# Borx25/CPU-Raytracing-experiments

Hardware: AMD Instinct MI355X
Metric: Mray/s (primary+bounce) (higher is better)
Workload: dtype f32; 1 GPU; cfg4: 4096x4096 px, S(100000) spheres + SAH BVH, MIS, Policy.max_bounces=9 (primary+8 bounces), 5 buckets, 64 accumulations/step; fixed image, tile rows split over the GPUs; image=4096x4096, spheres=100000, max_bounces=9, buckets=5, parallelism=single GPU, batches_in_flight=1, accumulations_per_batch=63, accumulations_per_batch_limit=63

## Files before the change

### cpu-raytracing-experiments_amd/csrc/kernels.hpp

```cpp
#pragma once
#include <hip/hip_runtime.h>
#include <stdint.h>
#include "device_math.hpp"

namespace mirt {

constexpr uint32_t kBlock = 256;
constexpr uint32_t kShadeBlock = 512;
constexpr uint32_t kTraceBlock = 1024;
constexpr uint32_t kLdsStack = 16;
constexpr uint32_t kLdsStackWide = 12;
constexpr uint32_t kLeafBit = 0x80000000u;
constexpr uint32_t kTileSize = 256;
constexpr uint32_t kTileRoot = 16;
constexpr uint32_t kStack = 64;
constexpr uint32_t kDestAccum = 0x80000000u;

struct SceneDev {
	const float4* recs;
	const float4* spheres;
	const int32_t* prim_mat;
	const float4* light_sphere;
	const float4* light_emit;
	const float4* mat_albedo;
// ... 6 lines not shown
	uint32_t wide;
	uint32_t chunk_max;
	uint32_t leaf_batch;
	uint32_t refill_idle;
	uint32_t stack16;
	float ambient[3];
	int32_t hdri_w, hdri_h;
	float hdri_fw, hdri_fh;
	uint32_t has_ambient;
	uint32_t use_bvh;
};

struct StreamBuf {
	float *px, *py, *pz, *dx, *dy, *dz;
	float *tr, *tg, *tb;
	float *rr, *rg, *rb;
	uint32_t* path;
};
struct ShadowBuf {
	float *px, *py, *pz;
	float *dx, *dy, *dz, *tfar;
	float *sr, *sg, *sb;
	float *rr, *rg, *rb;
	float *er, *eg, *eb;
	uint32_t* dest;
};
struct FrameParams {
	CameraParams cam;
	uint32_t h_tiles;
	uint32_t first_tile;
	uint32_t run_tiles;
	uint32_t stride_tiles;
	uint32_t n_pix;
	uint32_t pix_bits;
	uint32_t pix_mask;
	uint32_t acc_base;
	uint32_t batch_n;
	uint32_t idx_base;
	uint32_t idx_buckets;
	uint32_t max_bounces;
	uint32_t buckets;
	uint32_t mis;
	uint32_t n_lights;
	uint32_t first_groups;
	float inv_n_pix, inv_h_tiles, inv_run_tiles;
};
struct alignas(8) HitRec { float tfar; int32_t prim; };
struct DevCounters {
	unsigned long long rays, shadow_rays, nodes, spheres, shadow_nodes, shadow_spheres, terminated, dropped;
};

MIRT_DI uint32_t lane_id() { return __builtin_amdgcn_mbcnt_hi(~0u, __builtin_amdgcn_mbcnt_lo(~0u, 0u)); }
MIRT_DI uint32_t mask_rank(unsigned long long m) {
	return __builtin_amdgcn_mbcnt_hi(static_cast<uint32_t>(m >> 32), __builtin_amdgcn_mbcnt_lo(static_cast<uint32_t>(m), 0u));
// ... 526 lines not shown
	const bool all = bvh_all_in_lds(sc);
	if (sc.half_boxes && sc.wide) {
		if (!sc.stack16) trace_persistent<MODE, COUNT, false, true, false, true>(sc, tl, q, n, work_next, fat, c_nodes, c_spheres, load_ray, store_result, col);
		else if (all) trace_persistent<MODE, COUNT, true, true, true, true>(sc, tl, q, n, work_next, fat, c_nodes, c_spheres, load_ray, store_result, col);
		else trace_persistent<MODE, COUNT, false, true, true, true>(sc, tl, q, n, work_next, fat, c_nodes, c_spheres, load_ray, store_result, col);
	} else if (sc.half_boxes) {
		if (!sc.stack16) trace_persistent<MODE, COUNT, false, true, false, false>(sc, tl, q, n, work_next, fat, c_nodes, c_spheres, load_ray, store_result, col);
		else if (all) trace_persistent<MODE, COUNT, true, true, true, false>(sc, tl, q, n, work_next, fat, c_nodes, c_spheres, load_ray, store_result, col);
		else trace_persistent<MODE, COUNT, false, true, true, false>(sc, tl, q, n, work_next, fat, c_nodes, c_spheres, load_ray, store_result, col);
	} else {
		if (all) trace_persistent<MODE, COUNT, true, false, false, false>(sc, tl, q, n, work_next, fat, c_nodes, c_spheres, load_ray, store_result, col);
		else trace_persistent<MODE, COUNT, false, false, false, false>(sc, tl, q, n, work_next, fat, c_nodes, c_spheres, load_ray, store_result, col);
	}
}

MIRT_DI size_t accum_index(uint32_t acc_base, uint32_t buckets, uint32_t pix_bits, uint32_t path) {
	const uint32_t slot = path >> pix_bits;
	const uint32_t pix = path & ((1u << pix_bits) - 1u);
	const uint32_t bucket = (acc_base + slot + 1u) % buckets;
	return (static_cast<size_t>(pix >> 8) * buckets + bucket) * 3u * kTileSize + (pix & 255u);
}
MIRT_DI size_t accum_index(const FrameParams& fp, uint32_t path) { return accum_index(fp.idx_base, fp.idx_buckets, fp.pix_bits, path); }
MIRT_DI void accumulate_add(float* __restrict__ accum, size_t idx, float r, float g, float b) {
	accum[idx] += r; accum[idx + kTileSize] += g; accum[idx + 2 * kTileSize] += b;
}
constexpr uint32_t kIdxContrib = 0xffffffffu;
MIRT_DI size_t contrib_index(uint32_t batch_n, uint32_t pix_bits, uint32_t path) {
	const uint32_t slot = path >> pix_bits;
	const uint32_t pix = path & ((1u << pix_bits) - 1u);
	return ((static_cast<size_t>(pix >> 8) * batch_n + slot) * kTileSize + (pix & 255u)) * 3u;
}
MIRT_DI void path_result(float* __restrict__ accum, uint32_t idx_base, uint32_t idx_buckets, uint32_t pix_bits, uint32_t path, float r, float g, float b) {
	if (idx_base == kIdxContrib) {
		float* w = accum + contrib_index(idx_buckets, pix_bits, path);
		w[0] = 0.0f + r; w[1] = 0.0f + g; w[2] = 0.0f + b;
	} else accumulate_add(accum, accum_index(idx_base, idx_buckets, pix_bits, path), r, g, b);
}
MIRT_DI void path_result_add(float* __restrict__ accum, uint32_t idx_base, uint32_t idx_buckets, uint32_t pix_bits, uint32_t path, float r, float g, float b) {
	if (idx_base == kIdxContrib) {
		float* w = accum + contrib_index(idx_buckets, pix_bits, path);
		w[0] += r; w[1] += g; w[2] += b;
	} else accumulate_add(accum, accum_index(idx_base, idx_buckets, pix_bits, path), r, g, b);
}
MIRT_DI void path_result(float* __restrict__ accum, const FrameParams& fp, uint32_t path, float r, float g, float b) { path_result(accum, fp.idx_base, fp.idx_buckets, fp.pix_bits, path, r, g, b); }
constexpr uint32_t kDestFull = 0x40000000u;
constexpr uint32_t kDestSlot = 0x3fffffffu;
struct ShadowSink {
	float *rr, *rg, *rb;
	const float *px, *py, *pz;
	float* accum;
	uint32_t acc_base, buckets, pix_bits;
	uint32_t* occ;
};
MIRT_DI void shadow_origin(const ShadowBuf& sh, const ShadowSink& sink, uint32_t i, float& px, float& py, float& pz) {
	if (sink.occ) { px = sh.px[i]; py = sh.py[i]; pz = sh.pz[i]; return; }
	const uint32_t dw = sh.dest[i];
	if (dw & kDestAccum) { px = sh.px[i]; py = sh.py[i]; pz = sh.pz[i]; }
	else { const uint32_t d = dw & kDestSlot; px = sink.px[d]; py = sink.py[d]; pz = sink.pz[d]; }
}
MIRT_DI void shadow_finish(const ShadowBuf& sh, const ShadowSink& sink, uint32_t i, bool occluded, uint32_t& c_term) {
	if (sink.occ) { sink.occ[i] = occluded ? 1u : 0u; return; }
	const uint32_t dw = sh.dest[i];
	const uint32_t dest = dw & (kDestSlot | kDestAccum);
	if (dw & kDestAccum) c_term++;
	if (dw & kDestFull) {
		f3 R{ sh.rr[i], sh.rg[i], sh.rb[i] };
		const f3 E{ sh.er[i], sh.eg[i], sh.eb[i] };
		if (!occluded) { R.x += sh.sr[i]; R.y += sh.sg[i]; R.z += sh.sb[i]; }
		R.x += E.x; R.y += E.y; R.z += E.z;
		if (dest & kDestAccum) path_result(sink.accum, sink.acc_base, sink.buckets, sink.pix_bits, dest & ~kDestAccum, R.x, R.y, R.z);
		else { sink.rr[dest] = R.x; sink.rg[dest] = R.y; sink.rb[dest] = R.z; }
	} else if (!occluded) {
		const f3 S{ sh.sr[i], sh.sg[i], sh.sb[i] };
		if (dest & kDestAccum) path_result_add(sink.accum, sink.acc_base, sink.buckets, sink.pix_bits, dest & ~kDestAccum, S.x, S.y, S.z);
		else { sink.rr[dest] += S.x; sink.rg[dest] += S.y; sink.rb[dest] += S.z; }
	}
}

constexpr int kPrimaryNone = 0, kPrimaryAll = 1, kPrimaryList = 2;
MIRT_DI uint32_t primary_list_ray(const FrameParams& fp, const uint32_t* __restrict__ ov_pix, uint32_t n_ov, float inv_n_ov, uint32_t j) {
	uint32_t k;
	const uint32_t slot = udiv_f(j, n_ov, inv_n_ov, k);
	return slot * fp.n_pix + ov_pix[k];
}
template <bool COUNT, int PRIMARY>
__global__ __launch_bounds__(kTraceBlock, 8) void k_trace(SceneDev sc, FrameParams fp,
                                                       StreamBuf in, HitRec* __restrict__ hit_out,
                                                       Queue closest_queue, uint32_t* closest_work,
                                                       ShadowBuf sh, ShadowSink sink,
                                                       Queue shadow_queue, uint32_t* shadow_work, FatList fat_closest, FatList fat_shadow,
                                                       DevCounters* ctr) {
// ... 186 lines not shown

MIRT_DI uint32_t block_compact(bool flag, uint32_t value, uint32_t* scratch, uint32_t* list) {
	const unsigned long long m = __ballot(flag);
	const uint32_t wave = threadIdx.x >> 6, n_waves = blockDim.x >> 6;
	if (lane_id() == 0) scratch[wave] = static_cast<uint32_t>(__popcll(m));
	__syncthreads();
	uint32_t before = 0, total = 0;
	for (uint32_t w = 0; w < n_waves; w++) { const uint32_t c = scratch[w]; before += (w < wave) ? c : 0u; total += c; }
	if (flag) list[before + mask_rank(m)] = value;
	__syncthreads();
	return total;
}

template <bool FIRST, bool GGX>
__global__ __launch_bounds__(kShadeBlock, 6) void k_shade(SceneDev sc, FrameParams fp, StreamBuf in, const HitRec* __restrict__ hit_in, StreamBuf out, ShadowBuf sh, uint32_t bounce,
                                                  Queue in_queue, Queue next_queue, Queue shadow_queue, float* __restrict__ accum, DevCounters* ctr,
                                                  const float4* __restrict__ mat_ggx, float gloss_decay) {
	const QueueView qin = FIRST ? queue_identity(fp.n_pix * fp.batch_n) : queue_view(in_queue);
	const uint32_t n = qin.pre[kSegs];
	const uint32_t n_chunks = (fp.n_pix + kShadeBlock - 1u) / kShadeBlock;
	const bool last_bounce = !(bounce < fp.max_bounces - 1u);
	const float light_selection_pdf = 1.0f / static_cast<float>(fp.n_lights);
	__shared__ uint32_t append_scratch[72];
	__shared__ uint32_t compact_scratch[17];
	__shared__ uint32_t hit_list[kShadeBlock];
	__shared__ float4 s_albedo[MIRT_MAX_MATERIALS + 1], s_emission[MIRT_MAX_MATERIALS + 1];
	uint32_t c_term = 0, c_drop = 0, parity = 0;
	const uint32_t n_units = n_chunks * fp.first_groups;
	if (FIRST ? blockIdx.x >= n_units : blockIdx.x * kShadeBlock >= n) return;
	for (uint32_t m = threadIdx.x; m < sc.n_mat; m += kShadeBlock) { s_albedo[m] = GGX ? mat_ggx[m] : sc.mat_albedo[m]; s_emission[m] = sc.mat_emission[m]; }
	__syncthreads();
// ... 8 lines not shown
	for (uint32_t base = blockIdx.x * kShadeBlock; FIRST ? unit < n_units : base < n; parity ^= 1u) {
		const bool new_unit = FIRST && slot_it == slot_end;
		if (new_unit) {
			chunk = unit / fp.first_groups;
			const uint32_t g = unit - chunk * fp.first_groups;
			slot_it = g * fp.batch_n / fp.first_groups; slot_end = (g + 1u) * fp.batch_n / fp.first_groups;
		}
		const uint32_t iteration = FIRST ? chunk * fp.batch_n + slot_it : base / kShadeBlock;
		bool is_hit = false;
		uint32_t my_slot = next_slot;
		int32_t my_prim = next_prim;
		float my_tfar = 0.0f;
		f3 my_D{0, 0, 0};
		uint32_t my_path = 0u;
		bool lane_on;
		if (FIRST) {
			if (new_unit) {
				pix = chunk * kShadeBlock + threadIdx.x;
				if (pix < fp.n_pix) {
					uint32_t tile;
					pixel_xy(fp, pix, tile, pix_x, pix_y);
					pix_seed = (tile * kTileSize + (pix & 255u)) * (fp.max_bounces * 2u + 1u);
				}
			}
			lane_on = pix < fp.n_pix;
			my_slot = slot_it * fp.n_pix + pix;
			if (lane_on) {
				uint32_t rng = hash_2d(fp.acc_base + slot_it + 1u, pix_seed);
				const float s0 = rand_unit_float(rng);
				const float s1 = rand_unit_float(rng);
// ... 2 lines not shown
				{ const HitRec h = hit_in[my_slot]; my_prim = h.prim; my_tfar = h.tfar; }
			}
			if (++slot_it == slot_end) unit += gridDim.x;
		} else {
			lane_on = base + threadIdx.x < n;
			const uint32_t nb = base + gridDim.x * kShadeBlock;
			next_slot = (nb + threadIdx.x < n) ? queue_slot(qin, nb, nb + threadIdx.x) : 0u;
			next_prim = hit_in[next_slot].prim;
			base = nb;
		}
		{
			if (lane_on) {
				const uint32_t i = my_slot;
				const int32_t prim = my_prim;
				if (prim < 0) {
					f3 R{0.0f, 0.0f, 0.0f};
					float thr_x = 1.0f;
					uint32_t mpath = my_path; f3 md = my_D;
					if (!FIRST) { R = { in.rr[i], in.rg[i], in.rb[i] }; thr_x = in.tr[i]; mpath = in.path[i]; }
					if (sc.has_ambient) {
						if (!FIRST) md = { in.dx[i], in.dy[i], in.dz[i] };
						const f3 sky = sky_eval(sc, md.x, md.y, md.z);
						R.x += thr_x * sky.x; R.y += thr_x * sky.y; R.z += thr_x * sky.z;
					}
					path_result(accum, fp, mpath, R.x + 0.0f, R.y + 0.0f, R.z + 0.0f);
					c_term++;
				} else if (last_bounce) {
					c_drop++;
					if (fp.idx_base == kIdxContrib) {
						float* w = accum + contrib_index(fp.idx_buckets, fp.pix_bits, FIRST ? my_path : in.path[i]);
						w[0] = 0.0f; w[1] = 0.0f; w[2] = 0.0f;
					}
				} else is_hit = true;
			}
		}
		const uint32_t n_hits = FIRST ? 0u : block_compact(is_hit, my_slot, compact_scratch, hit_list);

		bool survive = false, has_shadow = false, terminated = false, has_E = false;
		uint32_t path = 0;
		f3 P{0, 0, 0}, ndir{0, 0, 0}, L{0, 0, 0}, srad{0, 0, 0}, E{0, 0, 0};
		f3 R{0.0f, 0.0f, 0.0f}, thr{1.0f, 1.0f, 1.0f};
		float light_distance = 0.0f;
		if (FIRST ? is_hit : threadIdx.x < n_hits) {
			const uint32_t i = FIRST ? my_slot : hit_list[threadIdx.x];
			f3 D = my_D;
			path = my_path;
			if (!FIRST) { path = in.path[i]; D = { in.dx[i], in.dy[i], in.dz[i] }; }
			float pdf_in = 0.0f;
			if (!FIRST) {
				R = { in.rr[i], in.rg[i], in.rb[i] };
				thr = { in.tr[i], in.tg[i], in.tb[i] };
				pdf_in = GGX ? 0.0f : MIRT_INV_PI * max_sel(0.0f, D.z);
			}
			const HitRec hrec = FIRST ? HitRec{ my_tfar, my_prim } : hit_in[i];
			const int32_t prim = hrec.prim;
			{
				const float depth = hrec.tfar;
				const float4 hs = sc.spheres[prim];
				const int32_t mat = sc.prim_mat[prim];
				const f3 O = FIRST ? f3{ fp.cam.pos[0], fp.cam.pos[1], fp.cam.pos[2] } : f3{ in.px[i], in.py[i], in.pz[i] };
				const f3 hit{ O.x + D.x * depth, O.y + D.y * depth, O.z + D.z * depth };
				f3 N = normalize3(f3{ hit.x - hs.x, hit.y - hs.y, hit.z - hs.z });
				if (dot3(N, D) >= 0.0f) N = f3{ -N.x, -N.y, -N.z };
				const quat T = tangent_space(N);
				const f3 Vl = to_local(T, f3{ -D.x, -D.y, -D.z });
// ... 77 lines not shown
					}
					const float q = 1.0f - max_sel(thr.x, max_sel(thr.y, thr.z));
					if (rand_unit_float(rng) < q) {
						terminated = true;
					} else {
						const float inv = 1.0f / max_sel(MIRT_FLT_EPSILON, 1.0f - q);
						thr = { thr.x * inv, thr.y * inv, thr.z * inv };
						ndir = to_world(T, sd);
						survive = true;
					}
				}
			}
		}
		uint32_t slot, sslot;
		block_append2(survive, has_shadow, next_queue, shadow_queue, iteration % kSegs, append_scratch, parity, slot, sslot);
		const bool direct = fp.idx_base != kIdxContrib;
		const bool full = has_shadow & (has_E | (terminated & direct));
		if (survive) {
			out.px[slot] = P.x; out.py[slot] = P.y; out.pz[slot] = P.z;
			out.dx[slot] = ndir.x; out.dy[slot] = ndir.y; out.dz[slot] = ndir.z;
			out.tr[slot] = thr.x; out.tg[slot] = thr.y; out.tb[slot] = thr.z;
			out.path[slot] = path;
		}
		if (has_shadow) {
			if (!survive) { sh.px[sslot] = P.x; sh.py[sslot] = P.y; sh.pz[sslot] = P.z; }
			sh.dx[sslot] = L.x; sh.dy[sslot] = L.y; sh.dz[sslot] = L.z;
			sh.tfar[sslot] = light_distance;
			sh.sr[sslot] = srad.x; sh.sg[sslot] = srad.y; sh.sb[sslot] = srad.z;
			if (full) {
				sh.rr[sslot] = R.x; sh.rg[sslot] = R.y; sh.rb[sslot] = R.z;
				sh.er[sslot] = E.x; sh.eg[sslot] = E.y; sh.eb[sslot] = E.z;
			}
			sh.dest[sslot] = (survive ? slot : (kDestAccum | path)) | (full ? kDestFull : 0u);
		}
		if ((survive | terminated) & !full) {
			const f3 Rf{ R.x + E.x, R.y + E.y, R.z + E.z };
			if (survive) { out.rr[slot] = Rf.x; out.rg[slot] = Rf.y; out.rb[slot] = Rf.z; }
			else path_result(accum, fp, path, Rf.x, Rf.y, Rf.z);
		}
		c_term += (terminated && !has_shadow) ? 1u : 0u;
	}
	wave_sum(c_term, &ctr->terminated);
	wave_sum(c_drop, &ctr->dropped);
}

__global__ __launch_bounds__(kBlock) void k_merge_contrib(float4* __restrict__ accum, const float4* __restrict__ contrib, uint32_t n_tiles, uint32_t buckets,
                                                          uint32_t batch_n, uint32_t acc_base) {
	constexpr uint32_t kQuads = kTileSize / 4u;
	const size_t n_items = static_cast<size_t>(n_tiles) * kQuads;
	const uint32_t first = min(buckets, batch_n);
	for (size_t item = static_cast<size_t>(blockIdx.x) * kBlock + threadIdx.x; item < n_items; item += static_cast<size_t>(gridDim.x) * kBlock) {
		const size_t tile = item / kQuads; const uint32_t q = static_cast<uint32_t>(item % kQuads);
		for (uint32_t k0 = 0; k0 < first; k0++) {
// ... 89 lines not shown
```

### cpu-raytracing-experiments_amd/csrc/mirt_capi.hip

```cpp
#include "../../include/mirt.h"
#include "kernels.hpp"
#include "bvh_layout.hpp"
#include "bvh_build.hpp"
#include "lbvh_build.hpp"

#include <hip/hip_runtime.h>
#include <algorithm>
#include <cstdarg>
#include <cstdio>
#include <cstdlib>
#include <cstring>
#include <string>
#include <vector>

using namespace mirt;

namespace {

thread_local std::string g_create_error;

struct DeviceBuffer {
	void* ptr = nullptr;
	size_t bytes = 0;
	hipError_t ensure(size_t want) {
// ... 76 lines not shown
};

namespace {

int fail(mirt_ctx* ctx, int code, const char* fmt, ...) {
	char buf[512];
	va_list ap; va_start(ap, fmt); vsnprintf(buf, sizeof buf, fmt, ap); va_end(ap);
	if (ctx) ctx->error = buf; else g_create_error = buf;
	return code;
}
#define HIP_TRY(ctx, expr) do { hipError_t _e = (expr); if (_e != hipSuccess) return fail(ctx, MIRT_ERR_HIP, "%s: %s", #expr, hipGetErrorString(_e)); } while (0)

constexpr uint32_t kMaxBatch = 256;
constexpr uint64_t kBatchRays = 1024ull << 20;
constexpr uint64_t kSerialRays = 96ull << 20;
constexpr size_t kStreamPlanes = 2 * 13 + 2 + 17;
uint32_t pix_bits_of(const mirt_ctx* c) { uint32_t b = 8; while ((1ull << b) < static_cast<uint64_t>(c->n_tiles) * kTileSize) b++; return b; }
uint32_t max_slots(const mirt_ctx* c) {
	const uint64_t n_pix = std::max<uint64_t>(static_cast<uint64_t>(c->n_tiles) * kTileSize, 1);
	const uint64_t by_slots = ((1ull << 30) - 3ull * kSegs * kShadeBlock) / n_pix;
	return static_cast<uint32_t>(std::max<uint64_t>(std::min<uint64_t>(std::min<uint64_t>(kMaxBatch, 1u << (30u - std::min<uint32_t>(pix_bits_of(c), 24u))), by_slots), 1));
}
uint32_t batch_floor(const mirt_ctx* c) { return std::max<uint32_t>(std::min<uint32_t>(c->policy.buckets, 5u), 1u); }
uint32_t batch_limit(const mirt_ctx* c) {
	if (c->policy.max_batch) return std::min(c->policy.max_batch, max_slots(c));
	const uint64_t n_pix = static_cast<uint64_t>(c->n_tiles) * kTileSize;
	if (n_pix == 0) return 1;
	const uint64_t b = std::max<uint64_t>((kBatchRays + n_pix / 2) / n_pix, batch_floor(c));
	return static_cast<uint32_t>(std::min<uint64_t>(std::min<uint64_t>(b, max_slots(c)), std::max<uint32_t>(c->batch_mem_cap, 1u)));
}
bool uses_contrib(const mirt_ctx* c, uint32_t n_slots) { return n_slots > 1 || batch_limit(c) > c->policy.buckets; }

uint32_t grid_for(const mirt_ctx* c, uint64_t work_items) {
	uint64_t blocks = (work_items + kBlock - 1) / kBlock;
	const uint64_t cap = static_cast<uint64_t>(c->n_cu) * 8u;
	if (blocks > cap) blocks = cap;
	if (blocks < 1) blocks = 1;
	return static_cast<uint32_t>(blocks);
}

constexpr uint32_t kLdsPerCu = 160u * 1024u;
struct LdsPlan {
	uint32_t stack16;
	uint32_t rec_bytes, lds_recs, lds_spheres, staged_bytes, stack_bytes;
	uint32_t launch_bytes;
	uint32_t wgs_per_cu;
// ... 39 lines not shown
	uint32_t* closest_work(uint32_t b) const { return word(b); }
	uint32_t* shadow_work(uint32_t b) const { return word(nb + b); }
	FatList fat_closest(uint32_t b, uint32_t* lists) const { return FatList{ word(2 * nb + b), lists, kFatCapacity }; }
	FatList fat_shadow(uint32_t b, uint32_t* lists) const { return FatList{ word(3 * nb + b), lists + kFatCapacity, kFatCapacity }; }
	uint32_t* cand_work() const { return word(4 * nb); }
	uint32_t* unused_fat_count() const { return word(4 * nb + 1); }
	uint32_t* listed_pixels() const { return word(4 * nb + 2); }
};
BatchCounters batch_counters(const mirt_ctx* c, const PipeSlot& sl) { return BatchCounters{ sl.counts.as<uint32_t>(), c->policy.max_bounces, c->seg_cap }; }
uint32_t wanted_slots(const mirt_ctx* c) {
	if (c->policy.streams) return std::min<uint32_t>(c->policy.streams, 8u);
	return static_cast<uint64_t>(c->n_tiles) * kTileSize * batch_limit(c) >= kSerialRays ? 1u : 3u;
}
uint64_t streams_bytes(const mirt_ctx* c) {
	const uint64_t rays = static_cast<uint64_t>(c->n_tiles) * kTileSize * batch_limit(c);
	return wanted_slots(c) * (rays * 4u * kStreamPlanes + (uses_contrib(c, wanted_slots(c)) ? rays * 12u : 0u));
}

void plan_batches(mirt_ctx* c) {
	const uint64_t n_pix = static_cast<uint64_t>(c->n_tiles) * kTileSize;
	if (c->policy.max_batch || n_pix == 0 || c->planned_for == n_pix) return;
	c->batch_mem_cap = kMaxBatch;
	size_t free_b = 0, total_b = 0, own = 0;
	for (const PipeSlot& sl : c->slots) own += sl.arena.bytes + sl.contrib.bytes;
	if (hipSetDevice(c->device) == hipSuccess && hipMemGetInfo(&free_b, &total_b) == hipSuccess)
		while (batch_limit(c) > batch_floor(c) && streams_bytes(c) > (free_b + own) / 5 * 4) c->batch_mem_cap = std::max(batch_limit(c) / 2, batch_floor(c));
	c->planned_for = n_pix;
}

int ensure_streams(mirt_ctx* c) {
	const uint64_t n_pix = static_cast<uint64_t>(c->n_tiles) * kTileSize;
	if (n_pix * batch_limit(c) == 0) return MIRT_OK;
	plan_batches(c);
	const uint64_t cap64 = n_pix * batch_limit(c);
	if (n_pix > (1u << 24)) return fail(c, MIRT_ERR_ARG, "more than 2^24 pixels per context (%llu); shard the tile range", (unsigned long long)n_pix);
	if (cap64 + 3ull * kSegs * kShadeBlock > (1ull << 30)) return fail(c, MIRT_ERR_ARG, "stream capacity %llu too large", (unsigned long long)cap64);
	const uint32_t seg_cap = static_cast<uint32_t>((((cap64 + kShadeBlock - 1) / kShadeBlock + kSegs - 1) / kSegs + 2) * kShadeBlock);
	const uint32_t cap = seg_cap * kSegs;
	const uint32_t nb = c->policy.max_bounces;
	const uint32_t want = wanted_slots(c);
	const bool contrib = uses_contrib(c, want);
	const size_t acc_bytes = static_cast<size_t>(c->n_tiles) * batch_limit(c) * 3 * kTileSize * sizeof(float);
	if (cap == c->capacity && nb == c->arena_bounces && c->slots.size() == want && (!contrib || c->slots[0].contrib.bytes >= acc_bytes)) return MIRT_OK;
	HIP_TRY(c, sync_all(c));
	while (c->slots.size() > want) {
		PipeSlot& sl = c->slots.back();
		sl.arena.release(); sl.counts.release(); sl.contrib.release(); sl.fat.release(); sl.cand.release();
		if (sl.batch_done) (void)hipEventDestroy(sl.batch_done);
		if (sl.merged) (void)hipEventDestroy(sl.merged);
		if (sl.stream) (void)hipStreamDestroy(sl.stream);
		c->slots.pop_back();
	}
	while (c->slots.size() < want) {
		PipeSlot sl;
		HIP_TRY(c, hipStreamCreateWithFlags(&sl.stream, hipStreamNonBlocking));
		HIP_TRY(c, hipEventCreateWithFlags(&sl.batch_done, hipEventDisableTiming));
		HIP_TRY(c, hipEventCreateWithFlags(&sl.merged, hipEventDisableTiming));
		c->slots.push_back(sl);
	}
	const size_t planes = kStreamPlanes;
	const size_t plane_bytes = (static_cast<size_t>(cap) * 4 + 255) & ~static_cast<size_t>(255);
	for (PipeSlot& sl : c->slots) {
		sl.in_use = false;
		hipError_t e = sl.arena.ensure(planes * plane_bytes);
		const char* what = "ray streams";
		if (e == hipSuccess) { e = sl.counts.ensure(BatchCounters::words(nb) * sizeof(uint32_t)); what = "queue counters"; }
		if (e == hipSuccess) { e = sl.fat.ensure(2u * kFatCapacity * sizeof(uint32_t)); what = "fat-ray lists"; }
		if (e == hipSuccess) { e = sl.cand.ensure(static_cast<size_t>(n_pix) * kCandStride * sizeof(uint32_t)); what = "candidate lists"; }
		if (e == hipSuccess) { if (contrib) { e = sl.contrib.ensure(acc_bytes); what = "contribution buffer"; } else sl.contrib.release(); }
		if (e != hipSuccess) {
			(void)hipGetLastError();
			if (e == hipErrorOutOfMemory && !c->policy.max_batch && batch_limit(c) > batch_floor(c)) {
				for (PipeSlot& other : c->slots) { other.arena.release(); other.contrib.release(); }
				c->capacity = 0;
				c->batch_mem_cap = std::max(batch_limit(c) / 2, batch_floor(c));
				return ensure_streams(c);
			}
			return fail(c, MIRT_ERR_HIP, "%s (%zu bytes of ray streams per batch in flight): %s", what, planes * plane_bytes, hipGetErrorString(e));
		}
		char* p = sl.arena.as<char>();
		auto take = [&]() { void* r = p; p += plane_bytes; return r; };
		for (int b = 0; b < 2; b++) {
			StreamBuf& s = sl.stream_buf[b];
			s.px = (float*)take(); s.py = (float*)take(); s.pz = (float*)take();
			s.dx = (float*)take(); s.dy = (float*)take(); s.dz = (float*)take();
			s.tr = (float*)take(); s.tg = (float*)take(); s.tb = (float*)take();
			s.rr = (float*)take(); s.rg = (float*)take(); s.rb = (float*)take();
			s.path = (uint32_t*)take();
		}
		sl.hit = (HitRec*)take(); (void)take();
		ShadowBuf& h = sl.shadow_buf;
		h.px = (float*)take(); h.py = (float*)take(); h.pz = (float*)take();
		h.dx = (float*)take(); h.dy = (float*)take(); h.dz = (float*)take(); h.tfar = (float*)take();
		h.sr = (float*)take(); h.sg = (float*)take(); h.sb = (float*)take();
		h.rr = (float*)take(); h.rg = (float*)take(); h.rb = (float*)take();
		h.er = (float*)take(); h.eg = (float*)take(); h.eb = (float*)take();
		h.dest = (uint32_t*)take();
	}
	c->capacity = cap;
	c->seg_cap = seg_cap;
	c->arena_bounces = nb;
	return MIRT_OK;
}

int alloc_accumulator(mirt_ctx* c) {
	const size_t floats = static_cast<size_t>(c->n_tiles) * c->policy.buckets * 3 * kTileSize;
	HIP_TRY(c, sync_all(c));
	HIP_TRY(c, c->accumulator.ensure(floats * sizeof(float)));
	if (floats) HIP_TRY(c, hipMemsetAsync(c->accumulator.ptr, 0, floats * sizeof(float), c->stream));
	HIP_TRY(c, hipMemsetAsync(c->counters.ptr, 0, sizeof(DevCounters), c->stream));
// ... 30 lines not shown
};

float bundle_half_angle(const mirt_ctx* c) { return (0.7072f / std::fabs(c->camera.z)) * 1.01f + 1e-4f; }

FrameParams frame_params(const mirt_ctx* c, uint32_t acc_base, uint32_t batch_n) {
	FrameParams fp{};
	fp.cam = c->camera;
	fp.h_tiles = c->h_tiles;
	fp.first_tile = c->first_tile;
	fp.run_tiles = c->run_tiles ? c->run_tiles : 1u;
	fp.stride_tiles = c->stride_tiles;
	fp.n_pix = c->n_tiles * kTileSize;
	fp.pix_bits = pix_bits_of(c); fp.pix_mask = (1u << fp.pix_bits) - 1u;
	fp.acc_base = acc_base;
	fp.batch_n = batch_n;
	fp.idx_base = acc_base;
	fp.idx_buckets = c->policy.buckets;
	fp.max_bounces = c->policy.max_bounces;
	fp.buckets = c->policy.buckets;
	fp.n_lights = c->scene.n_lights;
	fp.mis = (c->policy.mis && c->scene.n_lights > 0) ? 1u : 0u;
	fp.first_groups = 1;
	fp.inv_n_pix = fp.n_pix ? 1.0f / static_cast<float>(fp.n_pix) : 0.0f;
	fp.inv_h_tiles = fp.h_tiles ? 1.0f / static_cast<float>(fp.h_tiles) : 0.0f;
	fp.inv_run_tiles = 1.0f / static_cast<float>(fp.run_tiles);
	return fp;
}

SceneDev trace_scene(const mirt_ctx* c) {
	SceneDev sc = c->scene;
	sc.use_bvh = c->policy.use_bvh;
	sc.chunk_max = c->tune_chunk; sc.leaf_batch = c->tune_leaf_batch; sc.refill_idle = c->tune_refill_idle;
// ... 23 lines not shown
void launch_trace(const mirt_ctx* c, hipStream_t st, const SceneDev& sc, const FrameParams& fp, uint64_t n_rays, bool count, int primary, const TraceLaunch& t) {
	hipLaunchKernelGGL(kTrace[!count][primary], dim3(trace_grid(c, n_rays)), dim3(kTraceBlock), trace_lds(c), st, sc, fp, t.in, t.hit, t.closest_queue, t.closest_work,
	                   t.sh, t.sink, t.shadow_queue, t.shadow_work, t.fat_closest, t.fat_shadow, t.ctr);
	const uint32_t fat_grid = sc.n_spheres > 4096 ? static_cast<uint32_t>(c->n_cu) * 2u : 64u;
	if (sc.use_bvh) hipLaunchKernelGGL(kTraceFat[!count][primary], dim3(fat_grid), dim3(1024), 0, st, sc, fp, t.in, t.hit, t.fat_closest, t.sh, t.sink, t.fat_shadow, t.ctr, t.listed_pixels);
}

int launch_batch(mirt_ctx* c, uint32_t batch_n) {
	FrameParams fp = frame_params(c, c->accumulations, batch_n);
	const uint32_t nb = c->policy.max_bounces;
	const uint64_t total = static_cast<uint64_t>(fp.n_pix) * batch_n;
	if (total == 0) { c->accumulations += batch_n; return MIRT_OK; }
	const bool pipelined = c->slots.size() > 1;
	PipeSlot& sl = c->slots[c->batch_seq % c->slots.size()];
	hipStream_t st = pipelined ? sl.stream : c->stream;
	const bool contrib = uses_contrib(c, static_cast<uint32_t>(c->slots.size()));
	if (contrib) { fp.idx_base = kIdxContrib; fp.idx_buckets = batch_n; }
	const BatchCounters bc = batch_counters(c, sl);
	const float qn = c->camera.orient[0] * c->camera.orient[0] + c->camera.orient[1] * c->camera.orient[1] + c->camera.orient[2] * c->camera.orient[2] + c->camera.orient[3] * c->camera.orient[3];
	const bool bundle = c->policy.use_bvh && c->scene.n_recs != 0 && !c->policy.trace_primary_rays && batch_n >= 3 && c->camera.z != 0.0f && std::fabs(qn - 1.0f) < 1e-4f;
	DevCounters* ctr = c->counters.as<DevCounters>();
	const float4* mat_ggx = c->mat_ggx.as<float4>();
	float* accum = contrib ? sl.contrib.as<float>() : c->accumulator.as<float>();
	uint32_t* fat_lists = sl.fat.as<uint32_t>();
	const SceneDev sc = trace_scene(c);
	const bool count = c->policy.count_traffic != 0;
	const uint32_t sgrid = static_cast<uint32_t>(std::min<uint64_t>((total + kShadeBlock - 1) / kShadeBlock, static_cast<uint64_t>(c->n_cu) * c->tune_shade_wgs));
	{
		const uint64_t n_chunks = (static_cast<uint64_t>(fp.n_pix) + kShadeBlock - 1) / kShadeBlock;
		const uint64_t want = (8ull * sgrid + n_chunks - 1) / n_chunks;
		fp.first_groups = static_cast<uint32_t>(std::min<uint64_t>(std::max<uint64_t>(want, 1), batch_n));
	}

	if (pipelined && sl.in_use) HIP_TRY(c, hipStreamWaitEvent(st, sl.merged, 0));
	if (contrib && c->debug_poison_contrib)
		HIP_TRY(c, hipMemsetD32Async(reinterpret_cast<hipDeviceptr_t>(sl.contrib.ptr), 0x7fc0deadu, sl.contrib.bytes / sizeof(float), st));
	HIP_TRY(c, hipMemsetAsync(bc.w, 0, BatchCounters::words(nb) * sizeof(uint32_t), st));
	for (uint32_t bounce = 0; bounce < nb; bounce++) {
		const StreamBuf& in = sl.stream_buf[bounce & 1u];
		const StreamBuf& out = sl.stream_buf[(bounce & 1u) ^ 1u];
		const bool shadow_pending = fp.mis && bounce > 0;
		const bool lists = bounce == 0 && bundle;
		{ Bracket t(c, MIRT_K_TRACE, st);
		  if (lists) {
		    const FatList none{ bc.unused_fat_count(), fat_lists, 0u };
		    hipLaunchKernelGGL(kPrimaryCand[!count], dim3(trace_grid(c, fp.n_pix)), dim3(kTraceBlock), trace_lds(c), st, sc, fp, sl.cand.as<uint32_t>(), bundle_half_angle(c),
		                       bc.cand_work(), none, ctr, in.path, bc.listed_pixels());
		    const uint32_t hgrid = static_cast<uint32_t>(std::min<uint64_t>((static_cast<uint64_t>(fp.n_pix) + kBlock - 1) / kBlock, static_cast<uint64_t>(c->n_cu) * 64u));
		    hipLaunchKernelGGL(kPrimaryHits[!count], dim3(hgrid), dim3(kBlock), 0, st, sc, fp, sl.cand.as<uint32_t>(), sl.hit, ctr);
		  }
		  const ShadowSink sink{ in.rr, in.rg, in.rb, in.px, in.py, in.pz, accum, fp.idx_base, fp.idx_buckets, fp.pix_bits, nullptr };
		  const TraceLaunch tl{ in, sl.hit, lists ? Queue{ bc.listed_pixels(), 0u } : bc.stream_queue(bounce), bc.closest_work(bounce),
		                        sl.shadow_buf, sink, shadow_pending ? bc.shadow_queue(bounce - 1) : bc.empty_queue(), bc.shadow_work(shadow_pending ? bounce - 1 : 0),
		                        bc.fat_closest(bounce, fat_lists), bc.fat_shadow(bounce, fat_lists), bc.listed_pixels(), ctr };
		  launch_trace(c, st, sc, fp, total, count, lists ? kPrimaryList : bounce == 0 ? kPrimaryAll : kPrimaryNone, tl); }
		{ Bracket t(c, MIRT_K_SHADE, st);
		  const float decay = bounce < c->gloss_decay.size() ? c->gloss_decay[bounce] : 0.0f;
		  hipLaunchKernelGGL(kShade[bounce == 0][c->policy.brdf != 0], dim3(sgrid), dim3(kShadeBlock), 0, st, sc, fp, in, sl.hit, out, sl.shadow_buf, bounce,
		                     bc.stream_queue(bounce), bc.stream_queue(bounce + 1), bc.shadow_queue(bounce), accum, ctr, mat_ggx, decay); }
	}
	HIP_TRY(c, hipGetLastError());
	if (contrib) {
		if (pipelined) {
			HIP_TRY(c, hipEventRecord(sl.batch_done, st));
			HIP_TRY(c, hipStreamWaitEvent(c->stream, sl.batch_done, 0));
		}
		{ Bracket t(c, MIRT_K_RESOLVE);
		  hipLaunchKernelGGL(k_merge_contrib, dim3(grid_for(c, static_cast<uint64_t>(c->n_tiles) * (kTileSize / 4u))), dim3(kBlock), 0, c->stream,
		                     c->accumulator.as<float4>(), sl.contrib.as<float4>(), c->n_tiles, c->policy.buckets, batch_n, fp.acc_base); }
		HIP_TRY(c, hipGetLastError());
		if (pipelined) { HIP_TRY(c, hipEventRecord(sl.merged, c->stream)); sl.in_use = true; }
	}
	c->batch_seq++;
	c->accumulations += batch_n;
	if (c->policy.profile && c->pending.size() > 512) harvest(c);
	return MIRT_OK;
}

template <class T>
int upload(mirt_ctx* c, DeviceBuffer& buf, const std::vector<T>& host) {
	HIP_TRY(c, buf.ensure(std::max<size_t>(host.size(), 1) * sizeof(T)));
	if (!host.empty()) HIP_TRY(c, hipMemcpyAsync(buf.ptr, host.data(), host.size() * sizeof(T), hipMemcpyHostToDevice, c->stream));
	return MIRT_OK;
}

int check_ready(mirt_ctx* c) {
	if (!c) return MIRT_ERR_ARG;
// ... 576 lines not shown
```

Baseline: 8926 Mray/s.

## Write path radiance directly into per-batch contribution buffer, drop carried radiance planes

Removes the per-ray radiance planes (rr/rg/rb) from the stream and shadow buffers. Shade and shadow-finish kernels now add emission, sky and direct light straight into the per-sample contribution buffer, which is always allocated and merged. This cuts six float planes of stream traffic per bounce and removes the direct-accumulator path. In exchange it does scattered read-modify-write updates to the contribution buffer at every bounce, and the merge kernel now runs unconditionally.

```diff
diff --git a/cpu-raytracing-experiments_amd/csrc/kernels.hpp b/cpu-raytracing-experiments_amd/csrc/kernels.hpp
--- a/cpu-raytracing-experiments_amd/csrc/kernels.hpp
+++ b/cpu-raytracing-experiments_amd/csrc/kernels.hpp
@@ -44,14 +44,12 @@
 struct StreamBuf {
 	float *px, *py, *pz, *dx, *dy, *dz;
 	float *tr, *tg, *tb;
-	float *rr, *rg, *rb;
 	uint32_t* path;
 };
 struct ShadowBuf {
 	float *px, *py, *pz;
 	float *dx, *dy, *dz, *tfar;
 	float *sr, *sg, *sb;
-	float *rr, *rg, *rb;
 	float *er, *eg, *eb;
 	uint32_t* dest;
 };
@@ -66,8 +64,6 @@
 	uint32_t pix_mask;
 	uint32_t acc_base;
 	uint32_t batch_n;
-	uint32_t idx_base;
-	uint32_t idx_buckets;
 	uint32_t max_bounces;
 	uint32_t buckets;
 	uint32_t mis;
@@ -624,42 +620,18 @@
 	}
 }
 
-MIRT_DI size_t accum_index(uint32_t acc_base, uint32_t buckets, uint32_t pix_bits, uint32_t path) {
-	const uint32_t slot = path >> pix_bits;
-	const uint32_t pix = path & ((1u << pix_bits) - 1u);
-	const uint32_t bucket = (acc_base + slot + 1u) % buckets;
-	return (static_cast<size_t>(pix >> 8) * buckets + bucket) * 3u * kTileSize + (pix & 255u);
-}
-MIRT_DI size_t accum_index(const FrameParams& fp, uint32_t path) { return accum_index(fp.idx_base, fp.idx_buckets, fp.pix_bits, path); }
-MIRT_DI void accumulate_add(float* __restrict__ accum, size_t idx, float r, float g, float b) {
-	accum[idx] += r; accum[idx + kTileSize] += g; accum[idx + 2 * kTileSize] += b;
-}
-constexpr uint32_t kIdxContrib = 0xffffffffu;
 MIRT_DI size_t contrib_index(uint32_t batch_n, uint32_t pix_bits, uint32_t path) {
 	const uint32_t slot = path >> pix_bits;
 	const uint32_t pix = path & ((1u << pix_bits) - 1u);
 	return ((static_cast<size_t>(pix >> 8) * batch_n + slot) * kTileSize + (pix & 255u)) * 3u;
 }
-MIRT_DI void path_result(float* __restrict__ accum, uint32_t idx_base, uint32_t idx_buckets, uint32_t pix_bits, uint32_t path, float r, float g, float b) {
-	if (idx_base == kIdxContrib) {
-		float* w = accum + contrib_index(idx_buckets, pix_bits, path);
-		w[0] = 0.0f + r; w[1] = 0.0f + g; w[2] = 0.0f + b;
-	} else accumulate_add(accum, accum_index(idx_base, idx_buckets, pix_bits, path), r, g, b);
-}
-MIRT_DI void path_result_add(float* __restrict__ accum, uint32_t idx_base, uint32_t idx_buckets, uint32_t pix_bits, uint32_t path, float r, float g, float b) {
-	if (idx_base == kIdxContrib) {
-		float* w = accum + contrib_index(idx_buckets, pix_bits, path);
-		w[0] += r; w[1] += g; w[2] += b;
-	} else accumulate_add(accum, accum_index(idx_base, idx_buckets, pix_bits, path), r, g, b);
-}
-MIRT_DI void path_result(float* __restrict__ accum, const FrameParams& fp, uint32_t path, float r, float g, float b) { path_result(accum, fp.idx_base, fp.idx_buckets, fp.pix_bits, path, r, g, b); }
 constexpr uint32_t kDestFull = 0x40000000u;
 constexpr uint32_t kDestSlot = 0x3fffffffu;
 struct ShadowSink {
-	float *rr, *rg, *rb;
+	const uint32_t* path;
 	const float *px, *py, *pz;
-	float* accum;
-	uint32_t acc_base, buckets, pix_bits;
+	float* contrib;
+	uint32_t batch_n, pix_bits;
 	uint32_t* occ;
 };
 MIRT_DI void shadow_origin(const ShadowBuf& sh, const ShadowSink& sink, uint32_t i, float& px, float& py, float& pz) {
@@ -671,20 +643,15 @@
 MIRT_DI void shadow_finish(const ShadowBuf& sh, const ShadowSink& sink, uint32_t i, bool occluded, uint32_t& c_term) {
 	if (sink.occ) { sink.occ[i] = occluded ? 1u : 0u; return; }
 	const uint32_t dw = sh.dest[i];
-	const uint32_t dest = dw & (kDestSlot | kDestAccum);
 	if (dw & kDestAccum) c_term++;
-	if (dw & kDestFull) {
-		f3 R{ sh.rr[i], sh.rg[i], sh.rb[i] };
-		const f3 E{ sh.er[i], sh.eg[i], sh.eb[i] };
-		if (!occluded) { R.x += sh.sr[i]; R.y += sh.sg[i]; R.z += sh.sb[i]; }
-		R.x += E.x; R.y += E.y; R.z += E.z;
-		if (dest & kDestAccum) path_result(sink.accum, sink.acc_base, sink.buckets, sink.pix_bits, dest & ~kDestAccum, R.x, R.y, R.z);
-		else { sink.rr[dest] = R.x; sink.rg[dest] = R.y; sink.rb[dest] = R.z; }
-	} else if (!occluded) {
-		const f3 S{ sh.sr[i], sh.sg[i], sh.sb[i] };
-		if (dest & kDestAccum) path_result_add(sink.accum, sink.acc_base, sink.buckets, sink.pix_bits, dest & ~kDestAccum, S.x, S.y, S.z);
-		else { sink.rr[dest] += S.x; sink.rg[dest] += S.y; sink.rb[dest] += S.z; }
-	}
+	const bool full = (dw & kDestFull) != 0u;
+	if (occluded & !full) return;
+	const uint32_t path = (dw & kDestAccum) ? (dw & kDestSlot) : sink.path[dw & kDestSlot];
+	float* w = sink.contrib + contrib_index(sink.batch_n, sink.pix_bits, path);
+	f3 R{ w[0], w[1], w[2] };
+	if (!occluded) { R.x += sh.sr[i]; R.y += sh.sg[i]; R.z += sh.sb[i]; }
+	if (full) { R.x += sh.er[i]; R.y += sh.eg[i]; R.z += sh.eb[i]; }
+	w[0] = R.x; w[1] = R.y; w[2] = R.z;
 }
 
 constexpr int kPrimaryNone = 0, kPrimaryAll = 1, kPrimaryList = 2;
@@ -901,7 +868,7 @@
 
 template <bool FIRST, bool GGX>
 __global__ __launch_bounds__(kShadeBlock, 6) void k_shade(SceneDev sc, FrameParams fp, StreamBuf in, const HitRec* __restrict__ hit_in, StreamBuf out, ShadowBuf sh, uint32_t bounce,
-                                                  Queue in_queue, Queue next_queue, Queue shadow_queue, float* __restrict__ accum, DevCounters* ctr,
+                                                  Queue in_queue, Queue next_queue, Queue shadow_queue, float* __restrict__ contrib, DevCounters* ctr,
                                                   const float4* __restrict__ mat_ggx, float gloss_decay) {
 	const QueueView qin = FIRST ? queue_identity(fp.n_pix * fp.batch_n) : queue_view(in_queue);
 	const uint32_t n = qin.pre[kSegs];
@@ -940,6 +907,7 @@
 		f3 my_D{0, 0, 0};
 		uint32_t my_path = 0u;
 		bool lane_on;
+		f3 W0{0.0f, 0.0f, 0.0f};
 		if (FIRST) {
 			if (new_unit) {
 				pix = chunk * kShadeBlock + threadIdx.x;
@@ -972,21 +940,22 @@
 				const uint32_t i = my_slot;
 				const int32_t prim = my_prim;
 				if (prim < 0) {
-					f3 R{0.0f, 0.0f, 0.0f};
-					float thr_x = 1.0f;
-					uint32_t mpath = my_path; f3 md = my_D;
-					if (!FIRST) { R = { in.rr[i], in.rg[i], in.rb[i] }; thr_x = in.tr[i]; mpath = in.path[i]; }
 					if (sc.has_ambient) {
-						if (!FIRST) md = { in.dx[i], in.dy[i], in.dz[i] };
-						const f3 sky = sky_eval(sc, md.x, md.y, md.z);
-						R.x += thr_x * sky.x; R.y += thr_x * sky.y; R.z += thr_x * sky.z;
+						if (FIRST) {
+							const f3 sky = sky_eval(sc, my_D.x, my_D.y, my_D.z);
+							W0 = { 0.0f + 1.0f * sky.x, 0.0f + 1.0f * sky.y, 0.0f + 1.0f * sky.z };
+						} else {
+							const float thr_x = in.tr[i];
+							const f3 sky = sky_eval(sc, in.dx[i], in.dy[i], in.dz[i]);
+							float* w = contrib + contrib_index(fp.batch_n, fp.pix_bits, in.path[i]);
+							w[0] += thr_x * sky.x; w[1] += thr_x * sky.y; w[2] += thr_x * sky.z;
+						}
 					}
-					path_result(accum, fp, mpath, R.x + 0.0f, R.y + 0.0f, R.z + 0.0f);
 					c_term++;
 				} else if (last_bounce) {
 					c_drop++;
-					if (fp.idx_base == kIdxContrib) {
-						float* w = accum + contrib_index(fp.idx_buckets, fp.pix_bits, FIRST ? my_path : in.path[i]);
+					if (!FIRST) {
+						float* w = contrib + contrib_index(fp.batch_n, fp.pix_bits, in.path[i]);
 						w[0] = 0.0f; w[1] = 0.0f; w[2] = 0.0f;
 					}
 				} else is_hit = true;
@@ -997,7 +966,7 @@
 		bool survive = false, has_shadow = false, terminated = false, has_E = false;
 		uint32_t path = 0;
 		f3 P{0, 0, 0}, ndir{0, 0, 0}, L{0, 0, 0}, srad{0, 0, 0}, E{0, 0, 0};
-		f3 R{0.0f, 0.0f, 0.0f}, thr{1.0f, 1.0f, 1.0f};
+		f3 thr{1.0f, 1.0f, 1.0f};
 		float light_distance = 0.0f;
 		if (FIRST ? is_hit : threadIdx.x < n_hits) {
 			const uint32_t i = FIRST ? my_slot : hit_list[threadIdx.x];
@@ -1006,7 +975,6 @@
 			if (!FIRST) { path = in.path[i]; D = { in.dx[i], in.dy[i], in.dz[i] }; }
 			float pdf_in = 0.0f;
 			if (!FIRST) {
-				R = { in.rr[i], in.rg[i], in.rb[i] };
 				thr = { in.tr[i], in.tg[i], in.tb[i] };
 				pdf_in = GGX ? 0.0f : MIRT_INV_PI * max_sel(0.0f, D.z);
 			}
@@ -1114,8 +1082,7 @@
 		}
 		uint32_t slot, sslot;
 		block_append2(survive, has_shadow, next_queue, shadow_queue, iteration % kSegs, append_scratch, parity, slot, sslot);
-		const bool direct = fp.idx_base != kIdxContrib;
-		const bool full = has_shadow & (has_E | (terminated & direct));
+		const bool full = has_shadow & has_E;
 		if (survive) {
 			out.px[slot] = P.x; out.py[slot] = P.y; out.pz[slot] = P.z;
 			out.dx[slot] = ndir.x; out.dy[slot] = ndir.y; out.dz[slot] = ndir.z;
@@ -1127,16 +1094,19 @@
 			sh.dx[sslot] = L.x; sh.dy[sslot] = L.y; sh.dz[sslot] = L.z;
 			sh.tfar[sslot] = light_distance;
 			sh.sr[sslot] = srad.x; sh.sg[sslot] = srad.y; sh.sb[sslot] = srad.z;
-			if (full) {
-				sh.rr[sslot] = R.x; sh.rg[sslot] = R.y; sh.rb[sslot] = R.z;
-				sh.er[sslot] = E.x; sh.eg[sslot] = E.y; sh.eb[sslot] = E.z;
+			if (full) { sh.er[sslot] = E.x; sh.eg[sslot] = E.y; sh.eb[sslot] = E.z; }
+			sh.dest[sslot] = (survive ? slot : (kDestAccum | path)) | (full ? kDestFull : 0u);
+		}
+		if (has_E & !has_shadow) {
+			if (FIRST) W0 = { 0.0f + E.x, 0.0f + E.y, 0.0f + E.z };
+			else {
+				float* w = contrib + contrib_index(fp.batch_n, fp.pix_bits, path);
+				w[0] += E.x; w[1] += E.y; w[2] += E.z;
 			}
-			sh.dest[sslot] = (survive ? slot : (kDestAccum | path)) | (full ? kDestFull : 0u);
-		}
-		if ((survive | terminated) & !full) {
-			const f3 Rf{ R.x + E.x, R.y + E.y, R.z + E.z };
-			if (survive) { out.rr[slot] = Rf.x; out.rg[slot] = Rf.y; out.rb[slot] = Rf.z; }
-			else path_result(accum, fp, path, Rf.x, Rf.y, Rf.z);
+		}
+		if (FIRST && lane_on) {
+			float* w = contrib + contrib_index(fp.batch_n, fp.pix_bits, my_path);
+			w[0] = W0.x; w[1] = W0.y; w[2] = W0.z;
 		}
 		c_term += (terminated && !has_shadow) ? 1u : 0u;
 	}
diff --git a/cpu-raytracing-experiments_amd/csrc/mirt_capi.hip b/cpu-raytracing-experiments_amd/csrc/mirt_capi.hip
--- a/cpu-raytracing-experiments_amd/csrc/mirt_capi.hip
+++ b/cpu-raytracing-experiments_amd/csrc/mirt_capi.hip
@@ -114,7 +114,7 @@
 constexpr uint32_t kMaxBatch = 256;
 constexpr uint64_t kBatchRays = 1024ull << 20;
 constexpr uint64_t kSerialRays = 96ull << 20;
-constexpr size_t kStreamPlanes = 2 * 13 + 2 + 17;
+constexpr size_t kStreamPlanes = 2 * 10 + 2 + 14;
 uint32_t pix_bits_of(const mirt_ctx* c) { uint32_t b = 8; while ((1ull << b) < static_cast<uint64_t>(c->n_tiles) * kTileSize) b++; return b; }
 uint32_t max_slots(const mirt_ctx* c) {
 	const uint64_t n_pix = std::max<uint64_t>(static_cast<uint64_t>(c->n_tiles) * kTileSize, 1);
@@ -129,7 +129,6 @@
 	const uint64_t b = std::max<uint64_t>((kBatchRays + n_pix / 2) / n_pix, batch_floor(c));
 	return static_cast<uint32_t>(std::min<uint64_t>(std::min<uint64_t>(b, max_slots(c)), std::max<uint32_t>(c->batch_mem_cap, 1u)));
 }
-bool uses_contrib(const mirt_ctx* c, uint32_t n_slots) { return n_slots > 1 || batch_limit(c) > c->policy.buckets; }
 
 uint32_t grid_for(const mirt_ctx* c, uint64_t work_items) {
 	uint64_t blocks = (work_items + kBlock - 1) / kBlock;
@@ -199,7 +198,7 @@
 }
 uint64_t streams_bytes(const mirt_ctx* c) {
 	const uint64_t rays = static_cast<uint64_t>(c->n_tiles) * kTileSize * batch_limit(c);
-	return wanted_slots(c) * (rays * 4u * kStreamPlanes + (uses_contrib(c, wanted_slots(c)) ? rays * 12u : 0u));
+	return wanted_slots(c) * (rays * 4u * kStreamPlanes + rays * 12u);
 }
 
 void plan_batches(mirt_ctx* c) {
@@ -224,9 +223,8 @@
 	const uint32_t cap = seg_cap * kSegs;
 	const uint32_t nb = c->policy.max_bounces;
 	const uint32_t want = wanted_slots(c);
-	const bool contrib = uses_contrib(c, want);
 	const size_t acc_bytes = static_cast<size_t>(c->n_tiles) * batch_limit(c) * 3 * kTileSize * sizeof(float);
-	if (cap == c->capacity && nb == c->arena_bounces && c->slots.size() == want && (!contrib || c->slots[0].contrib.bytes >= acc_bytes)) return MIRT_OK;
+	if (cap == c->capacity && nb == c->arena_bounces && c->slots.size() == want && c->slots[0].contrib.bytes >= acc_bytes) return MIRT_OK;
 	HIP_TRY(c, sync_all(c));
 	while (c->slots.size() > want) {
 		PipeSlot& sl = c->slots.back();
@@ -252,7 +250,7 @@
 		if (e == hipSuccess) { e = sl.counts.ensure(BatchCounters::words(nb) * sizeof(uint32_t)); what = "queue counters"; }
 		if (e == hipSuccess) { e = sl.fat.ensure(2u * kFatCapacity * sizeof(uint32_t)); what = "fat-ray lists"; }
 		if (e == hipSuccess) { e = sl.cand.ensure(static_cast<size_t>(n_pix) * kCandStride * sizeof(uint32_t)); what = "candidate lists"; }
-		if (e == hipSuccess) { if (contrib) { e = sl.contrib.ensure(acc_bytes); what = "contribution buffer"; } else sl.contrib.release(); }
+		if (e == hipSuccess) { e = sl.contrib.ensure(acc_bytes); what = "contribution buffer"; }
 		if (e != hipSuccess) {
 			(void)hipGetLastError();
 			if (e == hipErrorOutOfMemory && !c->policy.max_batch && batch_limit(c) > batch_floor(c)) {
@@ -270,7 +268,6 @@
 			s.px = (float*)take(); s.py = (float*)take(); s.pz = (float*)take();
 			s.dx = (float*)take(); s.dy = (float*)take(); s.dz = (float*)take();
 			s.tr = (float*)take(); s.tg = (float*)take(); s.tb = (float*)take();
-			s.rr = (float*)take(); s.rg = (float*)take(); s.rb = (float*)take();
 			s.path = (uint32_t*)take();
 		}
 		sl.hit = (HitRec*)take(); (void)take();
@@ -278,7 +275,6 @@
 		h.px = (float*)take(); h.py = (float*)take(); h.pz = (float*)take();
 		h.dx = (float*)take(); h.dy = (float*)take(); h.dz = (float*)take(); h.tfar = (float*)take();
 		h.sr = (float*)take(); h.sg = (float*)take(); h.sb = (float*)take();
-		h.rr = (float*)take(); h.rg = (float*)take(); h.rb = (float*)take();
 		h.er = (float*)take(); h.eg = (float*)take(); h.eb = (float*)take();
 		h.dest = (uint32_t*)take();
 	}
@@ -339,8 +335,6 @@
 	fp.pix_bits = pix_bits_of(c); fp.pix_mask = (1u << fp.pix_bits) - 1u;
 	fp.acc_base = acc_base;
 	fp.batch_n = batch_n;
-	fp.idx_base = acc_base;
-	fp.idx_buckets = c->policy.buckets;
 	fp.max_bounces = c->policy.max_bounces;
 	fp.buckets = c->policy.buckets;
 	fp.n_lights = c->scene.n_lights;
@@ -394,14 +388,12 @@
 	const bool pipelined = c->slots.size() > 1;
 	PipeSlot& sl = c->slots[c->batch_seq % c->slots.size()];
 	hipStream_t st = pipelined ? sl.stream : c->stream;
-	const bool contrib = uses_contrib(c, static_cast<uint32_t>(c->slots.size()));
-	if (contrib) { fp.idx_base = kIdxContrib; fp.idx_buckets = batch_n; }
 	const BatchCounters bc = batch_counters(c, sl);
 	const float qn = c->camera.orient[0] * c->camera.orient[0] + c->camera.orient[1] * c->camera.orient[1] + c->camera.orient[2] * c->camera.orient[2] + c->camera.orient[3] * c->camera.orient[3];
 	const bool bundle = c->policy.use_bvh && c->scene.n_recs != 0 && !c->policy.trace_primary_rays && batch_n >= 3 && c->camera.z != 0.0f && std::fabs(qn - 1.0f) < 1e-4f;
 	DevCounters* ctr = c->counters.as<DevCounters>();
 	const float4* mat_ggx = c->mat_ggx.as<float4>();
-	float* accum = contrib ? sl.contrib.as<float>() : c->accumulator.as<float>();
+	float* contrib = sl.contrib.as<float>();
 	uint32_t* fat_lists = sl.fat.as<uint32_t>();
 	const SceneDev sc = trace_scene(c);
 	const bool count = c->policy.count_traffic != 0;
@@ -413,7 +405,7 @@
 	}
 
 	if (pipelined && sl.in_use) HIP_TRY(c, hipStreamWaitEvent(st, sl.merged, 0));
-	if (contrib && c->debug_poison_contrib)
+	if (c->debug_poison_contrib)
 		HIP_TRY(c, hipMemsetD32Async(reinterpret_cast<hipDeviceptr_t>(sl.contrib.ptr), 0x7fc0deadu, sl.contrib.bytes / sizeof(float), st));
 	HIP_TRY(c, hipMemsetAsync(bc.w, 0, BatchCounters::words(nb) * sizeof(uint32_t), st));
 	for (uint32_t bounce = 0; bounce < nb; bounce++) {
@@ -429,7 +421,7 @@
 		    const uint32_t hgrid = static_cast<uint32_t>(std::min<uint64_t>((static_cast<uint64_t>(fp.n_pix) + kBlock - 1) / kBlock, static_cast<uint64_t>(c->n_cu) * 64u));
 		    hipLaunchKernelGGL(kPrimaryHits[!count], dim3(hgrid), dim3(kBlock), 0, st, sc, fp, sl.cand.as<uint32_t>(), sl.hit, ctr);
 		  }
-		  const ShadowSink sink{ in.rr, in.rg, in.rb, in.px, in.py, in.pz, accum, fp.idx_base, fp.idx_buckets, fp.pix_bits, nullptr };
+		  const ShadowSink sink{ in.path, in.px, in.py, in.pz, contrib, batch_n, fp.pix_bits, nullptr };
 		  const TraceLaunch tl{ in, sl.hit, lists ? Queue{ bc.listed_pixels(), 0u } : bc.stream_queue(bounce), bc.closest_work(bounce),
 		                        sl.shadow_buf, sink, shadow_pending ? bc.shadow_queue(bounce - 1) : bc.empty_queue(), bc.shadow_work(shadow_pending ? bounce - 1 : 0),
 		                        bc.fat_closest(bounce, fat_lists), bc.fat_shadow(bounce, fat_lists), bc.listed_pixels(), ctr };
@@ -437,20 +429,18 @@
 		{ Bracket t(c, MIRT_K_SHADE, st);
 		  const float decay = bounce < c->gloss_decay.size() ? c->gloss_decay[bounce] : 0.0f;
 		  hipLaunchKernelGGL(kShade[bounce == 0][c->policy.brdf != 0], dim3(sgrid), dim3(kShadeBlock), 0, st, sc, fp, in, sl.hit, out, sl.shadow_buf, bounce,
-		                     bc.stream_queue(bounce), bc.stream_queue(bounce + 1), bc.shadow_queue(bounce), accum, ctr, mat_ggx, decay); }
+		                     bc.stream_queue(bounce), bc.stream_queue(bounce + 1), bc.shadow_queue(bounce), contrib, ctr, mat_ggx, decay); }
 	}
 	HIP_TRY(c, hipGetLastError());
-	if (contrib) {
-		if (pipelined) {
-			HIP_TRY(c, hipEventRecord(sl.batch_done, st));
-			HIP_TRY(c, hipStreamWaitEvent(c->stream, sl.batch_done, 0));
-		}
-		{ Bracket t(c, MIRT_K_RESOLVE);
-		  hipLaunchKernelGGL(k_merge_contrib, dim3(grid_for(c, static_cast<uint64_t>(c->n_tiles) * (kTileSize / 4u))), dim3(kBlock), 0, c->stream,
-		                     c->accumulator.as<float4>(), sl.contrib.as<float4>(), c->n_tiles, c->policy.buckets, batch_n, fp.acc_base); }
-		HIP_TRY(c, hipGetLastError());
-		if (pipelined) { HIP_TRY(c, hipEventRecord(sl.merged, c->stream)); sl.in_use = true; }
-	}
+	if (pipelined) {
+		HIP_TRY(c, hipEventRecord(sl.batch_done, st));
+		HIP_TRY(c, hipStreamWaitEvent(c->stream, sl.batch_done, 0));
+	}
+	{ Bracket t(c, MIRT_K_RESOLVE);
+	  hipLaunchKernelGGL(k_merge_contrib, dim3(grid_for(c, static_cast<uint64_t>(c->n_tiles) * (kTileSize / 4u))), dim3(kBlock), 0, c->stream,
+	                     c->accumulator.as<float4>(), sl.contrib.as<float4>(), c->n_tiles, c->policy.buckets, batch_n, fp.acc_base); }
+	HIP_TRY(c, hipGetLastError());
+	if (pipelined) { HIP_TRY(c, hipEventRecord(sl.merged, c->stream)); sl.in_use = true; }
 	c->batch_seq++;
 	c->accumulations += batch_n;
 	if (c->policy.profile && c->pending.size() > 512) harvest(c);
diff --git a/profiles/experiments/small_batches.py b/profiles/experiments/small_batches.py
--- /dev/null
+++ b/profiles/experiments/small_batches.py
@@ -0,0 +1,13 @@
+import importlib, os, sys, time
+ROOT = os.path.dirname(os.path.dirname(os.path.dirname(os.path.abspath(__file__))))
+sys.path.insert(0, ROOT)
+mirt = importlib.import_module("cpu-raytracing-experiments_amd")
+r = mirt.Renderer(mirt.scene.synthetic(1000, ambient=0.5), max_bounces=5, use_bvh=True, streams=1, max_batch=5); r.Resize(1024, 1024)
+r.Accumulate(10)
+for per_launch, launches in ((1, 200), (5, 80)):
+    for rep in range(3):
+        c0 = r.counters()["rays"]; t0 = time.perf_counter()
+        for _ in range(launches): r.Accumulate(per_launch)
+        dt = time.perf_counter() - t0
+        print(f"Accumulate({per_launch}) x {launches}: {dt / launches * 1e3:6.3f} ms per launch, {(r.counters()['rays'] - c0) / dt / 1e6:7.0f} Mray/s", flush=True)
+r.close()
```

Result: faster. 9317 Mray/s (median of 6 runs) (+4.4%).
